# JuliaReinforcementLearning/ReinforcementLearning.jl

Measured on NVIDIA H100. Metric: env-steps/sec at 65536 CartPole envs (full PPO iteration: rollout T=32 + GAE + 4 epochs x 4 minibatches), higher is better.
Workload: dtype f32

## Files before the change

reinforcementlearning.jl_b200/csrc/nn_tc.cu:

```cuda
#include "nn.cuh"
#include "perm.cuh"
#include "policy.cuh"
#include "tc_fwd.cuh"
#include "tc_split.h"
#include "wgmma.cuh"

namespace {

using tcfwd::G_F;
using tcfwd::GW_S;
using tcfwd::WIMG_BYTES;
using tcfwd::split2;
using tcfwd::wimg_off;
constexpr int TM = tcfwd::TM;
constexpr int H = tcfwd::H;
constexpr float kScaleW = tcfwd::kScale;

constexpr int NT7 = 512;
constexpr int kMaxStage = 10;
constexpr int GF_T = 128;
constexpr int GS_T = 16 * GF_T;
constexpr int FIMG = 8 * GS_T;
constexpr float kScaleH = 64.0f, kScaleX = 64.0f;
constexpr int kNo = 2;

struct SmemBwd {
    static_assert(FIMG % 128 == 0 && WIMG_BYTES % 128 == 0 && (2 * GS_T) % 16 == 0, "operand images must stay 128-byte aligned");
    alignas(128) uint8_t FP_full[FIMG];
    alignas(128) uint8_t FP_lo[FIMG];
    alignas(128) uint8_t FH_lo[FIMG];
    alignas(128) uint8_t FH_full[FIMG];
    alignas(128) uint8_t FQ_full[FIMG];
    alignas(128) uint8_t FQ_lo[FIMG];
    alignas(128) uint8_t B1[WIMG_BYTES];
    alignas(128) uint8_t XT[2][2 * GS_T];
    alignas(128) uint8_t AH_full[FIMG];
    alignas(128) uint8_t AH_lo[FIMG];
    alignas(16) float D[TM * H];
    uint64_t H1pos[2][TM];
    float W1[kInMax * H];
    float b1[H], b2[H];
    float W3[H * kNo];
    float b3[kNo];
    float Zp[4 * kNo * TM];
    float Red[32];
    double RedD[16];
    float step_scale;
    alignas(8) uint64_t bar1;
    alignas(8) uint64_t bar3;
    alignas(8) uint64_t bar4;
    float AccW2[64 * 65 + 64];
    float AccD4[64 * 9];
};
__device__ __forceinline__ int d_off(int s, int col) { return s * H + ((((col >> 2) ^ (s & 15))) << 2) + (col & 3); }
__device__ __forceinline__ void d_ld16(const float* D, int s, int f0, float (&v)[16]) {
#pragma unroll
    for (int u = 0; u < 4; ++u) {
        const float4 q4 = *reinterpret_cast<const float4*>(D + d_off(s, f0 + 4 * u));
        v[4 * u] = q4.x; v[4 * u + 1] = q4.y; v[4 * u + 2] = q4.z; v[4 * u + 3] = q4.w;
    }
}
template <int TB>
__device__ __forceinline__ void gemm_ts3(float (&d)[32], const uint8_t* a_hi, const uint8_t* a_lo, int h, uint64_t dB, uint32_t b_step) {
    const uint64_t dA = wg::make_desc(wg::smem_u32(a_hi) + 8 * h * GF_T, GS_T, GF_T), dAl = wg::make_desc(wg::smem_u32(a_lo) + 8 * h * GF_T, GS_T, GF_T);
    wg::fence();
#pragma unroll
    for (int k = 0; k < 4; ++k) {
        const uint32_t aa = k * 2 * GS_T, bb = k * b_step;
        wg::mma_m64n64k16<0, TB>(d, wg::desc_add(dA, aa), wg::desc_add(dB, bb), k ? 1u : 0u);
        wg::mma_m64n64k16<0, TB>(d, wg::desc_add(dA, aa), wg::desc_add(dB, 8 * GW_S + bb), 1u);
        wg::mma_m64n64k16<0, TB>(d, wg::desc_add(dAl, aa), wg::desc_add(dB, bb), 1u);
    }
    wg::commit();
    wg::wait_all();
}
__device__ __forceinline__ uint32_t fimg_off(int f, int s) { return (uint32_t)((f >> 3) * GS_T + (s >> 3) * GF_T + (s & 7) * 16 + (f & 7) * 2); }
__device__ __forceinline__ void store16_feat(uint8_t* img, int f0, int s, const uint32_t (&v)[8]) {
    uint8_t* p = img + fimg_off(f0, s);
    *reinterpret_cast<uint4*>(p) = make_uint4(v[0], v[1], v[2], v[3]);
    *reinterpret_cast<uint4*>(p + GS_T) = make_uint4(v[4], v[5], v[6], v[7]);
}
using b200perm::perm_index;
using b200perm::perm_index_bits;

__device__ __forceinline__ float lane_transpose_reduce32(float (&v)[32], int lane) {
#pragma unroll
    for (int st = 0; st < 5; ++st) {
        const int half = 16 >> st, off = 16 >> st;
        const bool upper = (lane & off) != 0;
#pragma unroll
        for (int n = 0; n < half; ++n) {
            float send = upper ? v[n] : v[n + half];
            float keep = upper ? v[n + half] : v[n];
            v[n] = keep + __shfl_xor_sync(0xffffffffu, send, off);
        }
    }
    return v[0];
}

__device__ __forceinline__ void worker_sync() { asm volatile("bar.sync 1, 512;" ::: "memory"); }
__device__ __forceinline__ void group_sync(int q) { asm volatile("bar.sync %0, 128;" ::"r"(5 + q) : "memory"); }
__device__ __forceinline__ void ready_arrive(int id) { asm volatile("bar.arrive %0, 640;" ::"r"(id) : "memory"); }
__device__ __forceinline__ void ready_wait(int id) { asm volatile("bar.sync %0, 640;" ::"r"(id) : "memory"); }
#ifdef B200RL_K7_TIMING
__device__ unsigned long long g_k7_phase[40];
__device__ int g_k7_watch = 0;
#define K7_T(i) do { if (tid == (g_k7_watch & 0xFFFF) && (int)blockIdx.x == (g_k7_watch >> 16)) { long long now_ = clock64(); g_k7_phase[i] += (unsigned long long)(now_ - tprev_); tprev_ = now_; } } while (0)
#else
#define K7_T(i) do { } while (0)
#endif
constexpr int NT7_ALL = NT7 + 128;
constexpr int kRegsMma = 64, kRegsWorker = 104;
static_assert(128 * kRegsMma + NT7 * kRegsWorker <= NT7_ALL * 96, "setmaxnreg split must fit the CTA's register allocation");
constexpr int kBarRdyA = 2, kBarRdyB = 3;
constexpr int kBarMma = 4;
__device__ __forceinline__ void mma_sync() { asm volatile("bar.sync %0, 128;" ::"n"(kBarMma) : "memory"); }

template <int ACT>
__global__ void __launch_bounds__(NT7_ALL, 1)
ac_loss_grad_tc_kernel(MlpDesc actor, MlpDesc critic, const float* params , AcHyper hp, AcBatch b, float* partial,
                       float* __restrict__ loss_partial, int64_t np_total, float scale_base ,
                       OptStep st ,
                       int n_actor ) {
    extern __shared__ __align__(1024) unsigned char smem_raw[];
    SmemBwd& sm = *reinterpret_cast<SmemBwd*>(smem_raw);
    const int role = (int)blockIdx.x < n_actor ? 0 : 1;
    const int cta = role ? (int)blockIdx.x - n_actor : (int)blockIdx.x;
    const int nctas = role ? (int)gridDim.x - n_actor : n_actor;
    const int nrows = max(n_actor, (int)gridDim.x - n_actor);
    const float scale_p = scale_base * (role ? 4.0f : 64.0f);
    const MlpDesc d = role ? critic : actor;
    const int act = ACT >= 0 ? ACT : d.act;
    const bool relu = act == B200RL_ACT_RELU;
    const int64_t poff = role ? actor.nparams() : 0;
    const float* __restrict__ p = params + poff;
    const int tid = threadIdx.x, warp = tid >> 5, lane = tid & 31;
    const int q = warp & 3, c = (warp >> 2) & 3;
    const int s = 32 * q + lane;
    {
        const float* b1 = p + (int64_t)H * d.in;
        const float* W2 = b1 + H;
        const float* b2 = W2 + (int64_t)H * H;
        const float s1 = relu ? kScaleH : 1.0f;
        for (int k = tid; k < kInMax * H; k += NT7_ALL) sm.W1[k] = (k / H) < d.in ? p[k] * s1 : 0.f;
        for (int k = tid; k < H; k += NT7_ALL) { sm.b1[k] = b1[k] * s1; sm.b2[k] = b2[k]; }
        for (int k = tid; k < H * kNo; k += NT7_ALL) {
            int j = k / kNo, o = k % kNo;
            sm.W3[k] = o < d.nout ? p[head_w<false>(d, o, j)] : 0.f;
        }
        if (tid < kNo) sm.b3[tid] = tid < d.nout ? p[head_b<false>(d, tid)] : 0.f;
        tcfwd::fill_w2_image<NT7_ALL>(sm.B1, W2);
    }
    if (tid == 32) {
        wg::mbar_init(&sm.bar1, 128); wg::mbar_init(&sm.bar3, 128); wg::mbar_init(&sm.bar4, 128);
    }
    wg::fence_proxy_async();
    __syncthreads();
    const float inv_s1 = 1.0f / (kScaleH * kScaleW), inv_s3 = 1.0f / (scale_p * kScaleH), inv_sp = 1.0f / scale_p, inv_s4 = 1.0f / (scale_p * kScaleX);
    const int64_t ntiles = (b.B + TM - 1) / TM;

    if (warp >= NT7 / 32) {
        asm volatile("setmaxnreg.dec.sync.aligned.u32 %0;" ::"n"(kRegsMma));
        const int t = tid - NT7, row0 = 16 * (t >> 5) + ((t & 31) >> 2), col0 = 2 * (t & 3);
        const uint64_t dB1k = wg::make_desc(wg::smem_u32(sm.B1), G_F, GW_S);
        const uint64_t dB1t = wg::make_desc(wg::smem_u32(sm.B1), GW_S, G_F);
        float dacc[32];
        auto store_d = [&](int h) {
#pragma unroll
            for (int j = 0; j < 8; ++j)
#pragma unroll
                for (int hh = 0; hh < 2; ++hh)
                    *reinterpret_cast<float2*>(sm.D + d_off(64 * h + row0 + 8 * hh, 8 * j + col0)) = make_float2(dacc[4 * j + 2 * hh], dacc[4 * j + 2 * hh + 1]);
        };
        auto gemm1 = [&](int h) { gemm_ts3<0>(dacc, sm.AH_full, sm.AH_lo, h, dB1k, 2 * G_F); };
        auto gemm2 = [&](int h) { gemm_ts3<1>(dacc, sm.FP_full, sm.FP_lo, h, dB1t, 2 * GW_S); };
        auto store_dp1 = [&](int h, int pbuf) {
#pragma unroll
            for (int hh = 0; hh < 2; ++hh) {
                const int ss = 64 * h + row0 + 8 * hh;
                const uint64_t pos = relu ? sm.H1pos[pbuf][ss] >> col0 : 0u;
#pragma unroll
                for (int j = 0; j < 8; ++j) {
                    const uint32_t off = fimg_off(8 * j + col0, ss);
                    float v0 = dacc[4 * j + 2 * hh] * (1.0f / kScaleW), v1 = dacc[4 * j + 2 * hh + 1] * (1.0f / kScaleW);
                    if (relu) {
                        v0 = ((pos >> (8 * j)) & 1u) ? v0 : 0.f;
                        v1 = ((pos >> (8 * j + 1)) & 1u) ? v1 : 0.f;
                    } else {
                        const float inv_h = 1.0f / kScaleH;
                        const float2 hf = __half22float2(*reinterpret_cast<const __half2*>(sm.FH_full + off));
                        const float2 lf = __half22float2(*reinterpret_cast<const __half2*>(sm.FH_lo + off));
                        v0 *= dact_f(act, (hf.x + lf.x) * inv_h);
                        v1 *= dact_f(act, (hf.y + lf.y) * inv_h);
                    }
                    uint32_t hi, lo;
                    split2(v0, v1, hi, lo);
                    *reinterpret_cast<uint32_t*>(sm.FQ_full + off) = hi;
                    *reinterpret_cast<uint32_t*>(sm.FQ_lo + off) = lo;
                }
            }
        };
        auto gemm3 = [&](int buf) {
            const uint64_t dPh = wg::make_desc(wg::smem_u32(sm.FP_full), GF_T, GS_T), dPl = wg::make_desc(wg::smem_u32(sm.FP_lo), GF_T, GS_T);
            const uint64_t dHh = wg::make_desc(wg::smem_u32(sm.FH_full), GF_T, GS_T), dHl = wg::make_desc(wg::smem_u32(sm.FH_lo), GF_T, GS_T);
            wg::fence();
#pragma unroll
            for (int k = 0; k < 8; ++k) {
                const uint32_t a = k * 2 * GF_T;
                wg::mma_m64n64k16<1, 1>(dacc, wg::desc_add(dPh, a), wg::desc_add(dHh, a), k ? 1u : 0u);
                wg::mma_m64n64k16<1, 1>(dacc, wg::desc_add(dPl, a), wg::desc_add(dHh, a), 1u);
                wg::mma_m64n64k16<1, 1>(dacc, wg::desc_add(dPh, a), wg::desc_add(dHl, a), 1u);
            }
            wg::commit();
            wg::wait_all();
#pragma unroll
            for (int j = 0; j < 8; ++j)
#pragma unroll
                for (int hh = 0; hh < 2; ++hh)
#pragma unroll
                    for (int e = 0; e < 2; ++e) sm.AccW2[(row0 + 8 * hh) * 65 + 8 * j + col0 + e] += dacc[4 * j + 2 * hh + e];
            const uint64_t dX = wg::make_desc(wg::smem_u32(sm.XT[buf]), GF_T, GS_T);
            float d8[4] = {0.f, 0.f, 0.f, 0.f};
            wg::fence();
#pragma unroll
            for (int k = 0; k < 8; ++k) {
                const uint32_t a = k * 2 * GF_T;
                wg::mma_m64n8k16<1, 1>(d8, wg::desc_add(dPh, a), wg::desc_add(dX, a), k ? 1u : 0u);
                wg::mma_m64n8k16<1, 1>(d8, wg::desc_add(dPl, a), wg::desc_add(dX, a), 1u);
            }
            wg::commit();
            wg::wait_all();
            if (col0 == 4) {
                sm.AccW2[64 * 65 + row0] += d8[0];
                sm.AccW2[64 * 65 + row0 + 8] += d8[2];
            }
        };
        auto gemm4 = [&](int buf) {
            const uint64_t dQh = wg::make_desc(wg::smem_u32(sm.FQ_full), GF_T, GS_T), dQl = wg::make_desc(wg::smem_u32(sm.FQ_lo), GF_T, GS_T);
            const uint64_t dX = wg::make_desc(wg::smem_u32(sm.XT[buf]), GF_T, GS_T);
            float d4[4] = {0.f, 0.f, 0.f, 0.f};
            wg::fence();
#pragma unroll
            for (int k = 0; k < 8; ++k) {
                const uint32_t a = k * 2 * GF_T;
                wg::mma_m64n8k16<1, 1>(d4, wg::desc_add(dQh, a), wg::desc_add(dX, a), k ? 1u : 0u);
                wg::mma_m64n8k16<1, 1>(d4, wg::desc_add(dQh, a), wg::desc_add(dX, GS_T + a), 1u);
                wg::mma_m64n8k16<1, 1>(d4, wg::desc_add(dQl, a), wg::desc_add(dX, a), 1u);
            }
            wg::commit();
            wg::wait_all();
#pragma unroll
            for (int hh = 0; hh < 2; ++hh)
#pragma unroll
                for (int e = 0; e < 2; ++e)
                    if (col0 + e < 5) sm.AccD4[(row0 + 8 * hh) * 9 + col0 + e] += d4[2 * hh + e];
        };
        if (cta < ntiles) {
            ready_wait(kBarRdyB);
            for (int h = 0; h < 2; ++h) { gemm1(h); store_d(h); }
            wg::mbar_arrive(&sm.bar1);
        }
        int buf = 0;
        for (int64_t tile = cta; tile < ntiles; tile += nctas, buf ^= 1) {
            ready_wait(kBarRdyA);
            for (int h = 0; h < 2; ++h) { gemm2(h); store_dp1(h, buf); }
            wg::fence_proxy_async();
            if (tile + nctas < ntiles) {
                ready_wait(kBarRdyB);
                for (int h = 0; h < 2; ++h) { gemm1(h); store_d(h); }
                wg::mbar_arrive(&sm.bar1);
            }
            gemm3(buf);
            wg::mbar_arrive(&sm.bar3);
            mma_sync();
            gemm4(buf);
            wg::mbar_arrive(&sm.bar4);
        }
    } else {
    asm volatile("setmaxnreg.inc.sync.aligned.u32 %0;" ::"n"(kRegsWorker));
    float g3[2][16];
    float gb3a0 = 0.f, gb3a1 = 0.f;
#pragma unroll
    for (int k = 0; k < 16; ++k) { g3[0][k] = 0.f; g3[1][k] = 0.f; }
    float l0 = 0.f, l1 = 0.f;
    float mean = 0.f, inv_std = 1.f;
    if (hp.normalize_adv && b.norm2) { mean = b.norm2[0]; inv_std = b.norm2[1]; }
    uint32_t ph1 = 0, ph3 = 0, ph4 = 0;
    bool gemm4_pending = false;
    int xbuf = 0;
    int pbuf = 0;
#ifdef B200RL_K7_TIMING
    long long tprev_ = clock64();
#endif
    const int pbits = b200perm::perm_bits(b.perm_n);
    const uint32_t pkey = ac_perm_key(b);
    auto index_of = [&](int64_t t) -> int32_t {
        const int64_t j = t * TM + s;
        if (t >= ntiles || j >= b.B) return -1;
        return b.idx ? b.idx[j] : (int32_t)perm_index_bits((uint32_t)(b.perm_offset + j), b.perm_n, pkey, pbits);
    };
    auto request = [&](int32_t g, float (&x)[kInMax], float (&a)[4]) {
#pragma unroll
        for (int k = 0; k < kInMax; ++k) { x[k] = 0.f; a[k] = 0.f; }
        if (g < 0) return;
        if (b.rec) {
            const float4 v0 = b.rec[2 * (int64_t)g], v1 = b.rec[2 * (int64_t)g + 1];
            x[0] = v0.x; x[1] = v0.y; x[2] = v0.z; x[3] = v0.w;
            a[0] = v1.x; a[1] = v1.y; a[2] = v1.z; a[3] = v1.w;
        } else {
#pragma unroll
            for (int i = 0; i < kInMax; ++i)
                if (i < b.ns) x[i] = b.states[(int64_t)b.ns * g + i];
            a[0] = reinterpret_cast<const float*>(b.actions)[g];
            a[1] = b.logp_old ? b.logp_old[g] : 0.f;
            a[2] = b.adv[g];
            a[3] = b.ret[g];
        }
    };
    float pfx[kInMax] = {0.f, 0.f, 0.f, 0.f}, pfa[4] = {0.f, 0.f, 0.f, 0.f};
    float aux[4] = {0.f, 0.f, 0.f, 0.f};
    int32_t gi_next = -1;
    bool gemm3_pending = false;
    float* const out = partial + (int64_t)cta * np_total + poff;
    float* const gW1 = out;
    float* const gb1 = out + (int64_t)H * d.in;
    float* const gW2 = gb1 + H;
    float* const gb2 = gW2 + (int64_t)H * H;
    for (int k = tid; k < 64 * 65 + 64; k += NT7) sm.AccW2[k] = 0.f;
    for (int k = tid; k < 64 * 9; k += NT7) sm.AccD4[k] = 0.f;
    float xo[kInMax];
    auto publish = [&](int64_t t) {
#pragma unroll
        for (int i = 0; i < kInMax; ++i) xo[i] = pfx[i];
        aux[0] = pfa[0];
        aux[1] = role == 0 ? pfa[1] : 0.f;
        aux[2] = role == 0 ? (hp.normalize_adv ? (pfa[2] - mean) * inv_std : pfa[2]) : 0.f;
        aux[3] = role == 0 ? 0.f : pfa[3];
        if (c == 0) {
            uint32_t h01, l01, h23, l23;
            split2(xo[0] * kScaleX, xo[1] * kScaleX, h01, l01);
            split2(xo[2] * kScaleX, xo[3] * kScaleX, h23, l23);
            uint8_t* xt = sm.XT[xbuf] + fimg_off(0, s);
            *reinterpret_cast<uint4*>(xt) = make_uint4(h01, h23, 0x3C00u, 0u);
            *reinterpret_cast<uint4*>(xt + GS_T) = make_uint4(l01, l23, 0u, 0u);
        }
        K7_T(16);
        xbuf ^= 1;
        request(gi_next, pfx, pfa);
        gi_next = index_of(t + 2 * nctas);
        K7_T(17);
    };
    auto layer1 = [&]() {
        uint32_t pos = 0;
        uint32_t hi8[8], lo8[8];
#pragma unroll
        for (int ch = 0; ch < 4; ++ch) {
            const int f0 = 16 * c + 4 * ch;
            float4 bb = *reinterpret_cast<const float4*>(sm.b1 + f0);
            float h[4] = {bb.x, bb.y, bb.z, bb.w};
#pragma unroll
            for (int k = 0; k < kInMax; ++k) {
                float4 w = *reinterpret_cast<const float4*>(sm.W1 + k * H + f0);
                h[0] = fmaf(w.x, xo[k], h[0]); h[1] = fmaf(w.y, xo[k], h[1]); h[2] = fmaf(w.z, xo[k], h[2]); h[3] = fmaf(w.w, xo[k], h[3]);
            }
            if (relu) {
#pragma unroll
                for (int e = 0; e < 4; ++e) { pos |= (h[e] > 0.f ? 1u : 0u) << (4 * ch + e); h[e] = fmaxf(h[e], 0.f); }
            } else {
#pragma unroll
                for (int e = 0; e < 4; ++e) h[e] = act_f(act, h[e]) * kScaleH;
            }
            split2(h[0], h[1], hi8[2 * ch], lo8[2 * ch]);
            split2(h[2], h[3], hi8[2 * ch + 1], lo8[2 * ch + 1]);
        }
        if (relu) reinterpret_cast<uint16_t*>(&sm.H1pos[pbuf][s])[c] = (uint16_t)pos;
        pbuf ^= 1;
        store16_feat(sm.AH_full, 16 * c, s, hi8);
        store16_feat(sm.AH_lo, 16 * c, s, lo8);
    };
    if (cta < ntiles) {
        request(index_of(cta), pfx, pfa);
        gi_next = index_of(cta + nctas);
        publish(cta);
        layer1();
        wg::fence_proxy_async();
        ready_arrive(kBarRdyB);
    }
#ifdef B200RL_K7_TIMING
    tprev_ = clock64();
#endif
    for (int64_t tile = cta; tile < ntiles; tile += nctas) {
        const bool has_next = tile + nctas < ntiles;
        wg::mbar_wait(&sm.bar1, ph1);
        ph1 ^= 1u;
        K7_T(0);
        float h2[16];
        {
            float v[16];
            d_ld16(sm.D, s, 16 * c, v);
            float zp[kNo] = {0.f, 0.f};
#pragma unroll
            for (int k = 0; k < 16; ++k) {
                const int f = 16 * c + k;
                h2[k] = act_f(act, fmaf(v[k], inv_s1, sm.b2[f]));
                float2 w = *reinterpret_cast<const float2*>(sm.W3 + f * kNo);
                zp[0] = fmaf(w.x, h2[k], zp[0]); zp[1] = fmaf(w.y, h2[k], zp[1]);
            }
#pragma unroll
            for (int o = 0; o < kNo; ++o) sm.Zp[(c * kNo + o) * TM + s] = zp[o];
        }
        K7_T(1);
        group_sync(q);
        K7_T(2);
        {
            float z[kNo];
#pragma unroll
            for (int o = 0; o < kNo; ++o)
                z[o] = sm.b3[o] + ((sm.Zp[o * TM + s] + sm.Zp[(kNo + o) * TM + s]) + (sm.Zp[(2 * kNo + o) * TM + s] + sm.Zp[(3 * kNo + o) * TM + s]));
            const bool valid = (tile * TM + s) < b.B;
            const policy::LossOut<kNo> lo_ = policy::sample_loss(actor.heads2, actor.nout, role, hp, b.inv_B, z, aux[0], aux[1], aux[2], aux[3]);
            float dz[kNo];
#pragma unroll
            for (int o = 0; o < kNo; ++o) dz[o] = valid ? lo_.dz[o] : 0.f;
            if (c == 0 && valid) { l0 += lo_.l0; l1 += lo_.l1; gb3a0 += dz[0]; gb3a1 += dz[1]; }
            const float dzs0 = dz[0] * scale_p, dzs1 = dz[1] * scale_p;
            float dp[16];
#pragma unroll
            for (int k = 0; k < 16; ++k) {
                const int f = 16 * c + k;
                float2 w = *reinterpret_cast<const float2*>(sm.W3 + f * kNo);
                const float dh = fmaf(w.x, dzs0, w.y * dzs1);
                dp[k] = relu ? (h2[k] > 0.f ? dh : 0.f) : dh * (1.f - h2[k] * h2[k]);
                g3[0][k] = fmaf(dz[0], h2[k], g3[0][k]);
                g3[1][k] = fmaf(dz[1], h2[k], g3[1][k]);
            }
            uint32_t hi8[8], lo8[8];
#pragma unroll
            for (int m = 0; m < 8; ++m) split2(dp[2 * m], dp[2 * m + 1], hi8[m], lo8[m]);
            K7_T(3);
            if (gemm3_pending) {
                wg::mbar_wait(&sm.bar3, ph3);
                ph3 ^= 1u;
                gemm3_pending = false;
            }
            K7_T(4);
            store16_feat(sm.FP_full, 16 * c, s, hi8);
            store16_feat(sm.FP_lo, 16 * c, s, lo8);
            {
                const uint32_t off = fimg_off(16 * c, s);
                const uint4 h0 = *reinterpret_cast<const uint4*>(sm.AH_full + off), h1 = *reinterpret_cast<const uint4*>(sm.AH_full + off + GS_T);
                const uint4 l0 = *reinterpret_cast<const uint4*>(sm.AH_lo + off), l1 = *reinterpret_cast<const uint4*>(sm.AH_lo + off + GS_T);
                *reinterpret_cast<uint4*>(sm.FH_full + off) = h0; *reinterpret_cast<uint4*>(sm.FH_full + off + GS_T) = h1;
                *reinterpret_cast<uint4*>(sm.FH_lo + off) = l0; *reinterpret_cast<uint4*>(sm.FH_lo + off + GS_T) = l1;
            }
        }
        K7_T(5);
        wg::fence_proxy_async();
        if (gemm4_pending) {
            wg::mbar_wait(&sm.bar4, ph4);
            ph4 ^= 1u;
        }
        K7_T(6);
        ready_arrive(kBarRdyA);
        gemm3_pending = true;
        gemm4_pending = true;
        K7_T(7);
        if (has_next) {
            publish(tile + nctas);
            layer1();
            wg::fence_proxy_async();
            K7_T(8);
            ready_arrive(kBarRdyB);
            K7_T(9);
        }
#ifdef B200RL_K7_TIMING
        if (tid == (g_k7_watch & 0xFFFF) && (int)blockIdx.x == (g_k7_watch >> 16)) g_k7_phase[15] += 1;
#endif
    }
    if (gemm3_pending) wg::mbar_wait(&sm.bar3, ph3);
    if (gemm4_pending) wg::mbar_wait(&sm.bar4, ph4);
    worker_sync();
    for (int k = tid; k < H * H; k += NT7) gW2[k] = sm.AccW2[(k & 63) * 65 + (k >> 6)] * inv_s3;
    if (tid < H) {
        gb2[tid] = sm.AccW2[64 * 65 + tid] * inv_sp;
        gb1[tid] = sm.AccD4[tid * 9 + 4] * inv_sp;
        for (int i = 0; i < d.in; ++i) gW1[tid + H * i] = sm.AccD4[tid * 9 + i] * inv_s4;
    }
    if (cta >= (int)gridDim.x - nctas) {
        const int64_t ooff = role ? 0 : actor.nparams(), on = role ? actor.nparams() : critic.nparams();
        float* orow = partial + (int64_t)cta * np_total + ooff;
        for (int64_t kk = tid; kk < on; kk += NT7) orow[kk] = 0.f;
    }
    float* red = reinterpret_cast<float*>(sm.FP_full);
    static_assert(offsetof(SmemBwd, XT) - offsetof(SmemBwd, FP_full) >= (2 * TM * 65 + 2 * 8 * 64) * 4, "drain scratch");
    {
        constexpr int RS = 65;
        float* seg = red + 2 * TM * RS;
#pragma unroll
        for (int k = 0; k < 16; ++k) {
            red[0 * TM * RS + s * RS + 16 * c + k] = g3[0][k];
            red[1 * TM * RS + s * RS + 16 * c + k] = g3[1][k];
        }
        worker_sync();
        {
            const int col = tid & 63, g = tid >> 6;
#pragma unroll
            for (int m = 0; m < 2; ++m) {
                float a = 0.f;
#pragma unroll
                for (int ss = 0; ss < 16; ++ss) a += red[m * TM * RS + (16 * g + ss) * RS + col];
                seg[(m * 8 + g) * 64 + col] = a;
            }
        }
        worker_sync();
        if (tid < 2 * H) {
            const int m = tid >> 6, col = tid & 63;
            float a = 0.f;
#pragma unroll
            for (int g = 0; g < 8; ++g) a += seg[(m * 8 + g) * 64 + col];
            if (m < d.nout) out[head_w<false>(d, m, col)] = a;
        }
        worker_sync();
    }
    if (c == 0) { red[s] = gb3a0; red[TM + s] = gb3a1; }
    worker_sync();
    if (warp < d.nout) {
        float a = (red[warp * TM + lane] + red[warp * TM + 32 + lane]) + (red[warp * TM + 64 + lane] + red[warp * TM + 96 + lane]);
#pragma unroll
        for (int o = 16; o > 0; o >>= 1) a += __shfl_xor_sync(0xffffffffu, a, o);
        if (lane == 0) out[head_b<false>(d, warp)] = a;
    }
    float t0 = l0, t1 = l1;
#pragma unroll
    for (int o = 16; o > 0; o >>= 1) { t0 += __shfl_xor_sync(0xffffffffu, t0, o); t1 += __shfl_xor_sync(0xffffffffu, t1, o); }
    worker_sync();
    if (lane == 0) { sm.Red[warp] = t0; sm.Red[16 + warp] = t1; }
    worker_sync();
    if (tid == 0) {
        float a0 = 0.f, a1 = 0.f;
        for (int k = 0; k < 16; ++k) { a0 += sm.Red[k]; a1 += sm.Red[16 + k]; }
        float* lp = loss_partial + (int64_t)blockIdx.x * 4;
        lp[0] = role ? 0.f : a0; lp[1] = role ? 0.f : a1; lp[2] = role ? a0 : 0.f; lp[3] = 0.f;
    }
    if (st.params) {
        const unsigned int G = gridDim.x;
        K7_T(24);
        worker_sync();
        K7_T(25);
        if (tid == 0) optim::grid_barrier(st.counters, G);
        worker_sync();
        K7_T(26);
        const int per = (int)((np_total + G - 1) / G);
        const int64_t k = (int64_t)blockIdx.x * per + tid;
        const bool mine = tid < per && k < np_total;
        const unsigned int seq = st.tab.nranks > 1 ? *st.seq_ptr + 1u : 0u;
        float* stage = reinterpret_cast<float*>(sm.FP_full);
        const int nstage = per * nrows;
        const int64_t k0 = (int64_t)blockIdx.x * per;
        {
            float t[kMaxStage];
#pragma unroll
            for (int j = 0; j < kMaxStage; ++j) {
                const int e = tid + j * NT7;
                const int row = e / per, col = e - row * per;
                t[j] = (e < nstage && k0 + col < np_total) ? __ldcg(partial + (int64_t)row * np_total + k0 + col) : 0.f;
            }
#pragma unroll
            for (int j = 0; j < kMaxStage; ++j) {
                const int e = tid + j * NT7;
                if (e < nstage) stage[e] = t[j];
            }
        }
        float* lstage = stage + nstage;
        if (blockIdx.x == 0) {
            float t[2];
#pragma unroll
            for (int j = 0; j < 2; ++j) t[j] = tid + j * NT7 < 4 * (int)G ? __ldcg(loss_partial + tid + j * NT7) : 0.f;
#pragma unroll
            for (int j = 0; j < 2; ++j) if (tid + j * NT7 < 4 * (int)G) lstage[tid + j * NT7] = t[j];
        }
        float m_k = 0.f, v_k = 0.f, p_k = 0.f;
        if (mine) { m_k = st.m[k]; v_k = st.v[k]; p_k = st.params[k]; }
        worker_sync();
        K7_T(27);
        float gk = 0.f;
        if (mine) {
            for (int c0 = 0; c0 < nrows; c0 += 8) {
                float t[8];
#pragma unroll
                for (int j = 0; j < 8; ++j) t[j] = c0 + j < nrows ? stage[(c0 + j) * per + tid] : 0.f;
#pragma unroll
                for (int j = 0; j < 8; ++j) if (c0 + j < nrows) gk += t[j];
            }
        }
        float lsum = 0.f;
        const bool loss_thread = blockIdx.x == 0 && tid < 4;
        if (loss_thread) {
            for (unsigned int c0 = 0; c0 < G; c0 += 8) {
                float t[8];
#pragma unroll
                for (int j = 0; j < 8; ++j) t[j] = c0 + j < G ? lstage[(c0 + j) * 4 + tid] : 0.f;
#pragma unroll
                for (int j = 0; j < 8; ++j) if (c0 + j < G) lsum += t[j];
            }
        }
        if (st.tab.nranks > 1) {
            const unsigned slot = seq & 1u;
            if (mine) p2p_push(st.tab, 0, slot, (size_t)k, __float_as_uint(gk), seq);
            if (loss_thread) p2p_push(st.tab, 0, slot, (size_t)np_total + tid, __float_as_uint(lsum), seq);
            if (mine) gk = p2p_sum_ranks(st.tab, 0, slot, (size_t)k, gk, seq);
            if (loss_thread) lsum = p2p_sum_ranks(st.tab, 0, slot, (size_t)np_total + tid, lsum, seq);
        }
        if (loss_thread) optim::publish_loss(st, tid, lsum);
        double sq = (double)gk * (double)gk;
#pragma unroll
        for (int o = 16; o > 0; o >>= 1) sq += __shfl_xor_sync(0xffffffffu, sq, o);
        if (lane == 0) sm.RedD[warp] = sq;
        worker_sync();
        K7_T(28);
        if (warp == 0) {
            if (lane == 0) {
                double t = 0.0;
                for (int w = 0; w < NT7 / 32; ++w) t += sm.RedD[w];
                st.cta_sumsq[blockIdx.x] = t;
                optim::grid_barrier(st.counters + 1, G);
            }
            __syncwarp();
            K7_T(29);
            double part[8];
#pragma unroll
            for (int j = 0; j < 8; ++j) part[j] = (unsigned)(lane + 32 * j) < G ? __ldcg(st.cta_sumsq + lane + 32 * j) : 0.0;
            double tot = 0.0;
#pragma unroll
            for (int j = 0; j < 8; ++j) tot += part[j];
#pragma unroll
            for (int o = 16; o > 0; o >>= 1) tot += __shfl_xor_sync(0xffffffffu, tot, o);
            if (lane == 0) {
                const float gn = (float)sqrt(tot);
                sm.step_scale = optim::clip_scale(gn, st.max_norm);
                if (blockIdx.x == 0) optim::publish_gnorm(st, gn);
            }
        }
        worker_sync();
        K7_T(30);
        const float bt1 = st.beta_t[0], bt2 = st.beta_t[1];
        if (mine) {
            gk *= sm.step_scale;
            st.grad[k] = gk;
            const optim::AdamOut a = optim::adam_update(gk, m_k, v_k, p_k, st.lr, st.b1, st.b2, st.eps, bt1, bt2);
            st.m[k] = a.m; st.v[k] = a.v; st.params[k] = a.p;
        }
        worker_sync();
        if (tid == 0) optim::close_step<3>(st, bt1, bt2, st.tab.nranks > 1, seq);
        K7_T(31);
    }
    }
    __syncthreads();
}

}

int nn_tc_actor_ctas(int grid, const MlpDesc& actor, const AcHyper& hp, int64_t ntiles) {
    static int forced = -2;
    if (forced == -2) { const char* e = getenv("B200RL_K7_ACTOR_CTAS"); forced = e ? atoi(e) : -1; }
    if (forced > 0 && forced < grid) return forced;
    (void)hp;
    return b200rl_tc_actor_ctas(grid, actor.heads2 != 0, ntiles);
}
int nn_tc_partial_rows(int grid, const MlpDesc& actor, const AcHyper& hp, int64_t B) {
    const int na = nn_tc_actor_ctas(grid, actor, hp, (B + TM - 1) / TM);
    return na > grid - na ? na : grid - na;
}
bool nn_tc_bwd_supported(const MlpDesc& actor, const MlpDesc& critic) {
    return actor.H == 64 && critic.H == 64 && actor.in <= kInMax && actor.nout <= 2 && critic.nout == 1;
}
bool nn_tc_step_fits(b200rl_ctx* ctx, int grid, const MlpDesc& actor, const AcHyper& hp, int64_t B, int64_t np) {
    const int64_t per = (np + grid - 1) / grid;
    return grid <= ctx->sm_count && grid <= 256 && per <= NT7 && per * nn_tc_partial_rows(grid, actor, hp, B) <= kMaxStage * NT7 &&
           4 * grid <= 2 * NT7;
}
int nn_tc_ac_loss_grad(b200rl_ctx* ctx, int grid, const MlpDesc& actor, const MlpDesc& critic, const float* params, const AcHyper& hp,
                       const AcBatch& b, float* partial, float* loss_partial, int64_t np, const OptStep* step) {
    const OptStep st = step ? *step : OptStep{};
    const int n_actor = nn_tc_actor_ctas(grid, actor, hp, (b.B + TM - 1) / TM);
    size_t smem = sizeof(SmemBwd) + 128;
    static unsigned long long attr_devices = 0;
    if (first_use_on_device(attr_devices, ctx->device)) {
        CUDA_TRY(cudaFuncSetAttribute(ac_loss_grad_tc_kernel<B200RL_ACT_RELU>, cudaFuncAttributeMaxDynamicSharedMemorySize, (int)smem));
        CUDA_TRY(cudaFuncSetAttribute(ac_loss_grad_tc_kernel<B200RL_ACT_TANH>, cudaFuncAttributeMaxDynamicSharedMemorySize, (int)smem));
        CUDA_TRY(cudaFuncSetAttribute(ac_loss_grad_tc_kernel<-1>, cudaFuncAttributeMaxDynamicSharedMemorySize, (int)smem));
    }
    const float scale_base = exp2f(floorf(log2f(1.0f / b.inv_B)));
    if (actor.act == critic.act && actor.act == B200RL_ACT_RELU)
        ac_loss_grad_tc_kernel<B200RL_ACT_RELU><<<grid, NT7_ALL, smem, ctx->stream>>>(actor, critic, params, hp, b, partial, loss_partial, np, scale_base, st, n_actor);
    else if (actor.act == critic.act && actor.act == B200RL_ACT_TANH)
        ac_loss_grad_tc_kernel<B200RL_ACT_TANH><<<grid, NT7_ALL, smem, ctx->stream>>>(actor, critic, params, hp, b, partial, loss_partial, np, scale_base, st, n_actor);
    else
        ac_loss_grad_tc_kernel<-1><<<grid, NT7_ALL, smem, ctx->stream>>>(actor, critic, params, hp, b, partial, loss_partial, np, scale_base, st, n_actor);
    LAUNCH_CHECK(ctx);
    return B200RL_OK;
}

#ifdef B200RL_K7_TIMING
extern "C" int b200rl_debug_k7_watch(int tid) {
    cudaDeviceSynchronize();
    return cudaMemcpyToSymbol(g_k7_watch, &tid, sizeof tid) == cudaSuccess ? 0 : -1;
}
extern "C" int b200rl_debug_k7_phases(unsigned long long* out16, int reset) {
    cudaDeviceSynchronize();
    if (cudaMemcpyFromSymbol(out16, g_k7_phase, sizeof(unsigned long long) * 40) != cudaSuccess) return -1;
    if (reset) { unsigned long long z[24] = {0}; cudaMemcpyToSymbol(g_k7_phase, z, sizeof z); }
    return 0;
}
#endif
```

Baseline: 309.5 million.

## Split worker-MMA handoff into per-half barriers and fuse gradient GEMMs

Worker warps are remapped so each row-half of the tile (64 samples) is handled by 256 threads. Each half gets its own named barriers (384 threads) and its own mbarrier, so the MMA warpgroup can start the layer-1/2 GEMMs for one half while the other half is still being produced. The separate weight-gradient GEMMs (gemm3, gemm4) are merged into one routine with a single mma_sync, cutting a synchronization point. Timing instrumentation gains MMA-side probes and atomic accumulation. In exchange the barrier protocol becomes more complex, and any mismatch in arrival counts could deadlock or race.

```diff
diff --git a/reinforcementlearning.jl_b200/csrc/nn_tc.cu b/reinforcementlearning.jl_b200/csrc/nn_tc.cu
--- a/reinforcementlearning.jl_b200/csrc/nn_tc.cu
+++ b/reinforcementlearning.jl_b200/csrc/nn_tc.cu
@@ -46,7 +46,7 @@
     float Red[32];
     double RedD[16];
     float step_scale;
-    alignas(8) uint64_t bar1;
+    alignas(8) uint64_t bar1[2];
     alignas(8) uint64_t bar3;
     alignas(8) uint64_t bar4;
     float AccW2[64 * 65 + 64];
@@ -100,19 +100,21 @@
 
 __device__ __forceinline__ void worker_sync() { asm volatile("bar.sync 1, 512;" ::: "memory"); }
 __device__ __forceinline__ void group_sync(int q) { asm volatile("bar.sync %0, 128;" ::"r"(5 + q) : "memory"); }
-__device__ __forceinline__ void ready_arrive(int id) { asm volatile("bar.arrive %0, 640;" ::"r"(id) : "memory"); }
-__device__ __forceinline__ void ready_wait(int id) { asm volatile("bar.sync %0, 640;" ::"r"(id) : "memory"); }
+__device__ __forceinline__ void ready_arrive(int id) { asm volatile("bar.arrive %0, 384;" ::"r"(id) : "memory"); }
+__device__ __forceinline__ void ready_wait(int id) { asm volatile("bar.sync %0, 384;" ::"r"(id) : "memory"); }
 #ifdef B200RL_K7_TIMING
 __device__ unsigned long long g_k7_phase[40];
 __device__ int g_k7_watch = 0;
-#define K7_T(i) do { if (tid == (g_k7_watch & 0xFFFF) && (int)blockIdx.x == (g_k7_watch >> 16)) { long long now_ = clock64(); g_k7_phase[i] += (unsigned long long)(now_ - tprev_); tprev_ = now_; } } while (0)
+#define K7_T(i) do { if (tid == (g_k7_watch & 0xFFFF) && (int)blockIdx.x == (g_k7_watch >> 16)) { long long now_ = clock64(); atomicAdd(&g_k7_phase[i], (unsigned long long)(now_ - tprev_)); tprev_ = now_; } } while (0)
+#define K7_M(i) do { if (tid == NT7 && (int)blockIdx.x == (g_k7_watch >> 16)) { long long now_ = clock64(); atomicAdd(&g_k7_phase[i], (unsigned long long)(now_ - mprev_)); mprev_ = now_; } } while (0)
 #else
 #define K7_T(i) do { } while (0)
+#define K7_M(i) do { } while (0)
 #endif
 constexpr int NT7_ALL = NT7 + 128;
 constexpr int kRegsMma = 64, kRegsWorker = 104;
 static_assert(128 * kRegsMma + NT7 * kRegsWorker <= NT7_ALL * 96, "setmaxnreg split must fit the CTA's register allocation");
-constexpr int kBarRdyA = 2, kBarRdyB = 3;
+constexpr int kBarRdyA = 9, kBarRdyB = 11;
 constexpr int kBarMma = 4;
 __device__ __forceinline__ void mma_sync() { asm volatile("bar.sync %0, 128;" ::"n"(kBarMma) : "memory"); }
 
@@ -135,8 +137,8 @@
     const int64_t poff = role ? actor.nparams() : 0;
     const float* __restrict__ p = params + poff;
     const int tid = threadIdx.x, warp = tid >> 5, lane = tid & 31;
-    const int q = warp & 3, c = (warp >> 2) & 3;
-    const int s = 32 * q + lane;
+    const int q = (warp >> 2) & 3, c = warp & 3;
+    const int s = 32 * q + lane, half = q >> 1;
     {
         const float* b1 = p + (int64_t)H * d.in;
         const float* W2 = b1 + H;
@@ -152,7 +154,7 @@
         tcfwd::fill_w2_image<NT7_ALL>(sm.B1, W2);
     }
     if (tid == 32) {
-        wg::mbar_init(&sm.bar1, 128); wg::mbar_init(&sm.bar3, 128); wg::mbar_init(&sm.bar4, 128);
+        wg::mbar_init(&sm.bar1[0], 128); wg::mbar_init(&sm.bar1[1], 128); wg::mbar_init(&sm.bar3, 128); wg::mbar_init(&sm.bar4, 128);
     }
     wg::fence_proxy_async();
     __syncthreads();
@@ -200,33 +202,39 @@
                 }
             }
         };
-        auto gemm3 = [&](int buf) {
+        auto gemm34 = [&](int buf) {
             const uint64_t dPh = wg::make_desc(wg::smem_u32(sm.FP_full), GF_T, GS_T), dPl = wg::make_desc(wg::smem_u32(sm.FP_lo), GF_T, GS_T);
-            const uint64_t dHh = wg::make_desc(wg::smem_u32(sm.FH_full), GF_T, GS_T), dHl = wg::make_desc(wg::smem_u32(sm.FH_lo), GF_T, GS_T);
-            wg::fence();
-#pragma unroll
-            for (int k = 0; k < 8; ++k) {
-                const uint32_t a = k * 2 * GF_T;
-                wg::mma_m64n64k16<1, 1>(dacc, wg::desc_add(dPh, a), wg::desc_add(dHh, a), k ? 1u : 0u);
-                wg::mma_m64n64k16<1, 1>(dacc, wg::desc_add(dPl, a), wg::desc_add(dHh, a), 1u);
-                wg::mma_m64n64k16<1, 1>(dacc, wg::desc_add(dPh, a), wg::desc_add(dHl, a), 1u);
-            }
-            wg::commit();
-            wg::wait_all();
+            {
+                const uint64_t dHh = wg::make_desc(wg::smem_u32(sm.FH_full), GF_T, GS_T), dHl = wg::make_desc(wg::smem_u32(sm.FH_lo), GF_T, GS_T);
+                wg::fence();
+#pragma unroll
+                for (int k = 0; k < 8; ++k) {
+                    const uint32_t a = k * 2 * GF_T;
+                    wg::mma_m64n64k16<1, 1>(dacc, wg::desc_add(dPh, a), wg::desc_add(dHh, a), k ? 1u : 0u);
+                    wg::mma_m64n64k16<1, 1>(dacc, wg::desc_add(dPl, a), wg::desc_add(dHh, a), 1u);
+                    wg::mma_m64n64k16<1, 1>(dacc, wg::desc_add(dPh, a), wg::desc_add(dHl, a), 1u);
+                }
+                wg::commit();
+                wg::wait_all();
+            }
 #pragma unroll
             for (int j = 0; j < 8; ++j)
 #pragma unroll
                 for (int hh = 0; hh < 2; ++hh)
 #pragma unroll
                     for (int e = 0; e < 2; ++e) sm.AccW2[(row0 + 8 * hh) * 65 + 8 * j + col0 + e] += dacc[4 * j + 2 * hh + e];
+            const uint64_t dQh = wg::make_desc(wg::smem_u32(sm.FQ_full), GF_T, GS_T), dQl = wg::make_desc(wg::smem_u32(sm.FQ_lo), GF_T, GS_T);
             const uint64_t dX = wg::make_desc(wg::smem_u32(sm.XT[buf]), GF_T, GS_T);
-            float d8[4] = {0.f, 0.f, 0.f, 0.f};
+            float d8[4] = {0.f, 0.f, 0.f, 0.f}, d4[4] = {0.f, 0.f, 0.f, 0.f};
             wg::fence();
 #pragma unroll
             for (int k = 0; k < 8; ++k) {
                 const uint32_t a = k * 2 * GF_T;
                 wg::mma_m64n8k16<1, 1>(d8, wg::desc_add(dPh, a), wg::desc_add(dX, a), k ? 1u : 0u);
                 wg::mma_m64n8k16<1, 1>(d8, wg::desc_add(dPl, a), wg::desc_add(dX, a), 1u);
+                wg::mma_m64n8k16<1, 1>(d4, wg::desc_add(dQh, a), wg::desc_add(dX, a), k ? 1u : 0u);
+                wg::mma_m64n8k16<1, 1>(d4, wg::desc_add(dQh, a), wg::desc_add(dX, GS_T + a), 1u);
+                wg::mma_m64n8k16<1, 1>(d4, wg::desc_add(dQl, a), wg::desc_add(dX, a), 1u);
             }
             wg::commit();
             wg::wait_all();
@@ -234,47 +242,47 @@
                 sm.AccW2[64 * 65 + row0] += d8[0];
                 sm.AccW2[64 * 65 + row0 + 8] += d8[2];
             }
-        };
-        auto gemm4 = [&](int buf) {
-            const uint64_t dQh = wg::make_desc(wg::smem_u32(sm.FQ_full), GF_T, GS_T), dQl = wg::make_desc(wg::smem_u32(sm.FQ_lo), GF_T, GS_T);
-            const uint64_t dX = wg::make_desc(wg::smem_u32(sm.XT[buf]), GF_T, GS_T);
-            float d4[4] = {0.f, 0.f, 0.f, 0.f};
-            wg::fence();
-#pragma unroll
-            for (int k = 0; k < 8; ++k) {
-                const uint32_t a = k * 2 * GF_T;
-                wg::mma_m64n8k16<1, 1>(d4, wg::desc_add(dQh, a), wg::desc_add(dX, a), k ? 1u : 0u);
-                wg::mma_m64n8k16<1, 1>(d4, wg::desc_add(dQh, a), wg::desc_add(dX, GS_T + a), 1u);
-                wg::mma_m64n8k16<1, 1>(d4, wg::desc_add(dQl, a), wg::desc_add(dX, a), 1u);
-            }
-            wg::commit();
-            wg::wait_all();
 #pragma unroll
             for (int hh = 0; hh < 2; ++hh)
 #pragma unroll
                 for (int e = 0; e < 2; ++e)
                     if (col0 + e < 5) sm.AccD4[(row0 + 8 * hh) * 9 + col0 + e] += d4[2 * hh + e];
         };
+#ifdef B200RL_K7_TIMING
+        long long mprev_ = clock64();
+#endif
         if (cta < ntiles) {
-            ready_wait(kBarRdyB);
-            for (int h = 0; h < 2; ++h) { gemm1(h); store_d(h); }
-            wg::mbar_arrive(&sm.bar1);
-        }
+            for (int h = 0; h < 2; ++h) {
+                ready_wait(kBarRdyB + h);
+                gemm1(h); store_d(h);
+                wg::mbar_arrive(&sm.bar1[h]);
+            }
+        }
+#ifdef B200RL_K7_TIMING
+        mprev_ = clock64();
+#endif
         int buf = 0;
         for (int64_t tile = cta; tile < ntiles; tile += nctas, buf ^= 1) {
-            ready_wait(kBarRdyA);
-            for (int h = 0; h < 2; ++h) { gemm2(h); store_dp1(h, buf); }
-            wg::fence_proxy_async();
-            if (tile + nctas < ntiles) {
-                ready_wait(kBarRdyB);
-                for (int h = 0; h < 2; ++h) { gemm1(h); store_d(h); }
-                wg::mbar_arrive(&sm.bar1);
-            }
-            gemm3(buf);
+            const bool has_next = tile + nctas < ntiles;
+            for (int h = 0; h < 2; ++h) {
+                ready_wait(kBarRdyA + h);
+                K7_M(18 + h);
+                gemm2(h); store_dp1(h, buf);
+                wg::fence_proxy_async();
+                K7_M(20 + h);
+                if (has_next) {
+                    ready_wait(kBarRdyB + h);
+                    K7_M(22 + h);
+                    gemm1(h); store_d(h);
+                    wg::mbar_arrive(&sm.bar1[h]);
+                    K7_M(32 + h);
+                }
+            }
+            mma_sync();
+            gemm34(buf);
             wg::mbar_arrive(&sm.bar3);
-            mma_sync();
-            gemm4(buf);
             wg::mbar_arrive(&sm.bar4);
+            K7_M(34);
         }
     } else {
     asm volatile("setmaxnreg.inc.sync.aligned.u32 %0;" ::"n"(kRegsWorker));
@@ -384,14 +392,14 @@
         publish(cta);
         layer1();
         wg::fence_proxy_async();
-        ready_arrive(kBarRdyB);
+        ready_arrive(kBarRdyB + half);
     }
 #ifdef B200RL_K7_TIMING
     tprev_ = clock64();
 #endif
     for (int64_t tile = cta; tile < ntiles; tile += nctas) {
         const bool has_next = tile + nctas < ntiles;
-        wg::mbar_wait(&sm.bar1, ph1);
+        wg::mbar_wait(&sm.bar1[half], ph1);
         ph1 ^= 1u;
         K7_T(0);
         float h2[16];
@@ -461,7 +469,7 @@
             ph4 ^= 1u;
         }
         K7_T(6);
-        ready_arrive(kBarRdyA);
+        ready_arrive(kBarRdyA + half);
         gemm3_pending = true;
         gemm4_pending = true;
         K7_T(7);
@@ -470,7 +478,7 @@
             layer1();
             wg::fence_proxy_async();
             K7_T(8);
-            ready_arrive(kBarRdyB);
+            ready_arrive(kBarRdyB + half);
             K7_T(9);
         }
 #ifdef B200RL_K7_TIMING
@@ -709,7 +717,7 @@
 extern "C" int b200rl_debug_k7_phases(unsigned long long* out16, int reset) {
     cudaDeviceSynchronize();
     if (cudaMemcpyFromSymbol(out16, g_k7_phase, sizeof(unsigned long long) * 40) != cudaSuccess) return -1;
-    if (reset) { unsigned long long z[24] = {0}; cudaMemcpyToSymbol(g_k7_phase, z, sizeof z); }
+    if (reset) { unsigned long long z[40] = {0}; cudaMemcpyToSymbol(g_k7_phase, z, sizeof z); }
     return 0;
 }
 #endif
```

Measured after the change: 315.4 million (median of 6 runs). 1.9% higher.
